# NHLBI/long_context_biomedical_imaging

Hardware: AMD Instinct MI355X
Metric: image-tokens/sec fwd+bwd, ViT patch=2 512^2 (L=65536), 1/2/4/8 MI355X (higher is better)
Workload: dtype bf16; 1 GPU; ViT-small p2 512x512 2-D seg (ViTUNETR head), full attention; global_batch=2, seq_len=65536, parallelism=ddp1, per_gpu_batch=2, optimizer=adam, loss=CrossEntropy, activation_checkpointing=none, hip_graph=False, tuned_gemms=True

## Files before the change

### include/lci.h

```cpp
#ifndef LCI_H_
#define LCI_H_

#ifdef __cplusplus
extern "C" {
#endif

#define LCI_ABI_VERSION 40
const char* lci_last_error(void);
int lci_abi_version(void);
const char* lci_build_hash(void);

int lci_attn_fwd(const void* qkv, void* out, float* lse2, float* knorm_ws, int B, int L, int H, int head_dim,
                 float scale, void* stream);
long long lci_attn_fwd_ws_bytes(int B, int L, int H);
int lci_attn_fwd_variant(int variant, const void* qkv, void* out, float* lse2, float* knorm_ws, int B, int L, int H,
                         int head_dim, float scale, void* stream);
int lci_attn_fwd_pick(int B, int L, int H, int n_cu);
int lci_attn_bwd(const void* qkv, const void* out, const void* dout, const float* lse2, void* dqkv,
                 float* delta_ws, int B, int L, int H, int head_dim, float scale, void* stream);
long long lci_attn_bwd_ws_bytes(int B, int H, int L);
int lci_attn_bwd_stage(int stage, const void* qkv, const void* out, const void* dout, const float* lse2,
                       void* dqkv, float* delta_ws, int B, int L, int H, int head_dim, float scale, void* stream);
int lci_attn_bwd_variant(int dq_variant, int stage, const void* qkv, const void* out, const void* dout,
                         const float* lse2, void* dqkv, float* delta_ws, int B, int L, int H, int head_dim,
                         float scale, void* stream);
int lci_attn_bwd_dq_pick(int B, int L, int H, int n_cu);

int lci_attn_gen_fwd(int dtype, const void* qkv, void* out, float* lse, int B, int L, int H, int head_dim,
                     float scale, void* stream);
int lci_attn_gen_bwd(int dtype, const void* qkv, const void* out, const void* dout, const float* lse, void* dqkv,
                     float* delta_ws, int B, int L, int H, int head_dim, float scale, void* stream);

long long lci_window_bias_elems(const int* geo, int has_mask);
int lci_window_bias(const float* rpb, const float* mask, void* bias, void* biasT, const int* geo, void* stream);
int lci_window_attn_fwd(const void* qkv, const float* qkv_bias, const void* biasT, int has_mask, void* out,
                        float* lse2, const int* geo, float scale, void* stream);
int lci_window_attn_bwd(const void* qkv, const float* qkv_bias, const void* bias, const void* biasT, int has_mask,
                        const void* out, const void* dout, const float* lse2, void* dqkv, float* dbias_pad,
                        float* pad_ws, void* dS, float* drpb, const int* geo, float scale, void* stream);
long long lci_window_dS_elems(const int* geo);
long long lci_window_pad_ws_elems(const int* geo);
int lci_window_bwd_needs_plain(const int* geo);
int lci_window_index_map(const int* geo, int* src_row, int* region, int* rid, int* wtype, void* stream);

int lci_window_gather(const void* src, void* dst, int elem_bytes, const int* geo, int scatter, void* stream);

int lci_conv3_fwd(const void* x, const void* w, void* y, int B, int D, int H, int W, int Cin, int Cout, int KD,
                  void* stream);
int lci_conv3_fwd_splits(long long V, int Cin, int Cout, int KD);
int lci_conv3_pack_weight(const float* w, void* out, int Cout, int Cin, int KD, int mode, int Cin_pad, void* stream);
int lci_convup_interleave(const void* src, void* dst, int B, int D, int H, int W, int kd, int kh, int kw, int C, int ld,
                          int adjoint, void* stream);
int lci_conv3_fwd_split(const void* x, const void* w, void* y, float* part, int nsplit, int B, int D, int H, int W,
                        int Cin, int Cout, int KD, void* stream);
long long lci_conv3_wgrad_splits(long long V, int Cin, int Cout, int KD);
int lci_conv3_wgrad(const void* x, const void* dy, float* part, int B, int D, int H, int W, int Cin, int Cout,
                    int KD, void* stream);

int lci_inorm_chunks(long long V, int B);
int lci_inorm_reduce(const void* x, const void* dz, const float* stats, float* part, long long V, int B, int C,
                     int act, float slope, void* stream);
int lci_inorm_finalize(const float* part, float* out, long long V, int B, int C, int mode, float eps, void* stream);
int lci_bn_relu_fwd(const void* x, const float* stats, const float* w, const float* b, float* y, long long V, int C,
                    void* stream);
int lci_bn_relu_bwd_reduce(const void* x, const void* dy, int dy_f32, const float* stats, const float* w,
                           const float* b, float* part, long long V, int C, void* stream);
int lci_bn_relu_bwd_apply(const void* x, const void* dy, int dy_f32, const float* stats, const float* coef,
                          const float* w, const float* b, void* dx, long long V, int C, void* stream);
int lci_inorm_apply(const void* x, const void* dz, const float* stats, const float* coef, void* out, long long V,
                    int B, int C, int act, float slope, void* stream);
int lci_inorm_apply_res(const void* x, const float* stats, const void* y, const float* stats_y, void* out,
                        long long V, int B, int C, float slope, void* stream);

int lci_selective_scan_fwd(int dtype, const void* u, const void* delta, const float* A, const void* Bm,
                           const void* Cm, const float* D, const float* delta_bias, void* y,
                           const long long* strides, int B, int L, int Dx, int N, int chunk, int delta_softplus,
                           float* xend, float* xinit, float* sdt, void* ckpt, void* stream);
int lci_selective_scan_bwd(int dtype, const void* u, const void* delta, const float* A, const void* Bm,
                           const void* Cm, const float* D, const float* delta_bias, const void* dy, void* du,
// ... 149 lines not shown
```

### long_context_biomedical_imaging_amd/csrc/attention.hip

```cpp
#include "common.hpp"

#include <type_traits>
#include <utility>

namespace lci {

constexpr int DH = 64;
constexpr int KT = 64;
constexpr float NEG_BIG = -1.0e30f;

struct AttnArgs {
  const bf16* q; const bf16* k; const bf16* v;
  const bf16* o; const bf16* dout;
  bf16* out;
  bf16* dk; bf16* dv;
  float* lse2;
  float* delta;
  long long bs_q, bs_k, bs_v, bs_o, bs_do, bs_out, bs_dk, bs_dv;
  int rs_q, rs_k, rs_v, rs_o, rs_do, rs_out, rs_dk, rs_dv;
  int hs;
  int H, L;
  float c;
  float scale;
};

__global__ __launch_bounds__(256) void attn_key_norm_kernel(AttnArgs a, float* knorm, int nkt) {
  const int lane = threadIdx.x & 63, t = blockIdx.x * 4 + (threadIdx.x >> 6);
  const int hh = blockIdx.y, b = blockIdx.z;
  if (t >= nkt) return;
  const int key = t * KT + lane;
  float ss = 0.f;
  if (key < a.L) {
    const bf16* kp = a.k + b * a.bs_k + (long long)key * a.rs_k + hh * a.hs;
#pragma unroll
    for (int c = 0; c < DH / 8; ++c) {
      const bf16x8 v = *(const bf16x8*)(kp + 8 * c);
#pragma unroll
      for (int j = 0; j < 8; ++j) ss += to_f32(v[j]) * to_f32(v[j]);
    }
  }
#pragma unroll
  for (int off = 32; off >= 1; off >>= 1) ss = fmaxf(ss, __shfl_xor(ss, off));
  if (lane == 0) knorm[((long long)b * a.H + hh) * nkt + t] = sqrtf(ss);
}

constexpr float SAFE_EXP2 = 64.f;
__global__ __launch_bounds__(256) void attn_bwd_delta_kernel(AttnArgs a) {
  const int tid = threadIdx.x;
  const int row = blockIdx.x * 32 + (tid >> 3), ch = tid & 7;
  const int hh = blockIdx.y, b = blockIdx.z;
  float acc = 0.f;
  if (row < a.L) {
    const bf16x8 o = *(const bf16x8*)(a.o + b * a.bs_o + (long long)row * a.rs_o + hh * a.hs + ch * 8);
    const bf16x8 d = *(const bf16x8*)(a.dout + b * a.bs_do + (long long)row * a.rs_do + hh * a.hs + ch * 8);
#pragma unroll
    for (int j = 0; j < 8; ++j) acc += to_f32(o[j]) * to_f32(d[j]);
  }
  acc += __shfl_xor(acc, 1);
  acc += __shfl_xor(acc, 2);
  acc += __shfl_xor(acc, 4);
  if (ch == 0 && row < a.L) {
    float* ws = a.delta + ((long long)b * a.H + hh) * 2 * a.L;
    ws[row] = -a.lse2[((long long)b * a.H + hh) * a.L + row];
    ws[a.L + row] = -acc;
  }
}

constexpr int HS_NW = 4;
__device__ __forceinline__ int sw128(int row, int col) {
  const int g = ((row >> 2) & 3) | (((row >> 1) & 1) << 2);
  return row * DH + ((((col >> 3) ^ g) << 3) | (col & 7));
}
__device__ __forceinline__ void hs_dma16(rsrc_t r, int voff, int soff, unsigned lds) {
  unsigned keep;
  asm volatile("s_mov_b32 %0, m0\n\ts_mov_b32 m0, %3\n\ts_nop 0\n\tbuffer_load_dwordx4 %1, %2, %4 offen lds\n\ts_mov_b32 m0, %0"
               : "=&s"(keep) : "v"(voff), "s"(r), "s"(lds), "s"(soff) : "memory");
}
__device__ __forceinline__ void hs_dma4(rsrc_t r, int voff, int soff, unsigned lds) {
  unsigned keep;
  asm volatile("s_mov_b32 %0, m0\n\ts_mov_b32 m0, %3\n\ts_nop 0\n\tbuffer_load_dword %1, %2, %4 offen lds\n\ts_mov_b32 m0, %0"
               : "=&s"(keep) : "v"(voff), "s"(r), "s"(lds), "s"(soff) : "memory");
}
__device__ __forceinline__ u32x4 hs_ld16(rsrc_t r, int voff, int soff) {
  u32x4 v;
  asm volatile("buffer_load_dwordx4 %0, %1, %2, %3 offen" : "=a"(v) : "v"(voff), "s"(r), "s"(soff) : "memory");
  return v;
}
__device__ __forceinline__ uint32_t hs_ld4(rsrc_t r, int voff, int soff) {
  uint32_t v;
  asm volatile("buffer_load_dword %0, %1, %2, %3 offen" : "=a"(v) : "v"(voff), "s"(r), "s"(soff) : "memory");
  return v;
}
template <int N>
__device__ __forceinline__ void hs_vmcnt() {
  __builtin_amdgcn_s_waitcnt((N & 15) | ((N >> 4) << 14) | (7 << 4) | (15 << 8));
}
#define HS_TO_AGPR(x) asm volatile("" : "=a"(x) : "0"(x))
#define HS_OPAQUE(x) asm volatile("" : "+v"(x))
#define HS_KEEP(x) asm volatile("" ::"v"(x))
#define HS_EXP(x) asm volatile("v_exp_f32 %0, %0" : "+v"(x))
#define HS_MUL(p, e) asm volatile("v_mul_f32 %0, %1, %0" : "+v"(p) : "v"(e))
#define HS_CVT(w, x0, x1) asm volatile("v_cvt_pk_bf16_f32 %0, %1, %2" : "=v"(w) : "v"(x0), "v"(x1))
#define HS_MFMA_G(acc, A, B) \
  asm volatile("v_mfma_f32_32x32x16_bf16 %0, %1, %2, %0" : "+a"(acc) : "v"(A), "v"(B))
#define HS_MFMA_C0(d, A, B, C) \
  asm volatile("v_mfma_f32_32x32x16_bf16 %0, %1, %2, %3" : "=&v"(d) : "v"(A), "a"(B), "v"(C))
#define HS_MFMA_C(d, A, B) \
  asm volatile("v_mfma_f32_32x32x16_bf16 %0, %1, %2, %0" : "+v"(d) : "v"(A), "a"(B))

constexpr unsigned LGKM0_WAIT = 0xC07F;
template <int OFF>
__device__ __forceinline__ void hs_st16(unsigned addr, const u32x4& v) {
  asm volatile("ds_write_b128 %0, %1 offset:%2" ::"v"(addr), "a"(v), "i"(OFF) : "memory");
}
template <int OFF>
__device__ __forceinline__ void hs_st4(unsigned addr, uint32_t v) {
  asm volatile("ds_write_b32 %0, %1 offset:%2" ::"v"(addr), "a"(v), "i"(OFF) : "memory");
}
__device__ __forceinline__ u32x4 hs_ld16v(rsrc_t r, int voff, int soff) {
  u32x4 v;
  asm volatile("buffer_load_dwordx4 %0, %1, %2, %3 offen" : "=v"(v) : "v"(voff), "s"(r), "s"(soff) : "memory");
  return v;
}
template <int OFF>
__device__ __forceinline__ void hs_st16v(unsigned addr, const u32x4& v) {
  asm volatile("ds_write_b128 %0, %1 offset:%2" ::"v"(addr), "v"(v), "i"(OFF) : "memory");
}
template <class F, int... G>
__device__ __forceinline__ void hs_for_gaps(F&& f, std::integer_sequence<int, G...>) {
  (f(std::integral_constant<int, G>{}), ...);
}

constexpr int HS_TILE_B = KT * DH * 2;
constexpr int HS_SLOT_B = 2 * HS_TILE_B;
constexpr int HS_NSLOT = 4;
static_assert((HS_NSLOT & (HS_NSLOT - 1)) == 0, "ring slot of tile t is t & (HS_NSLOT - 1)");
static_assert(HS_NSLOT * HS_SLOT_B == 65536, "ring reachable by DS immediates");

struct HsRing {
  rsrc_t rx, ry;
  int x0, x1, y0, y1;
  int rs2x, rs2y;
  unsigned lds0;
  int wave;
  static __device__ __forceinline__ int toff(int t, int rs2) { return (int)((uint32_t)t * KT * (uint32_t)rs2); }
  __device__ __forceinline__ rsrc_t rsrc(int i) const { return i < 2 ? rx : ry; }
  __device__ __forceinline__ int voff(int i) const { return i == 0 ? x0 : i == 1 ? x1 : i == 2 ? y0 : y1; }
  __device__ __forceinline__ int soff(int t, int i) const { return toff(t, i < 2 ? rs2x : rs2y); }
  __device__ __forceinline__ void dma(int t, int i) const {
    const unsigned sb = lds0 + (unsigned)((t & (HS_NSLOT - 1)) * HS_SLOT_B);
    hs_dma16(rsrc(i), voff(i), soff(t, i), sb + (i >> 1) * HS_TILE_B + 2048 * wave + (i & 1) * 1024);
  }
};
__device__ __forceinline__ rsrc_t hs_rows_rsrc(const bf16* p, int rs2, int L) {
  return make_rsrc(p, (uint32_t)(L - 1) * (uint32_t)rs2 + DH * 2);
}
__device__ __forceinline__ HsRing hs_ring(rsrc_t rx, int rs2x, rsrc_t ry, int rs2y, int lane, int wave,
                                          const char* smem) {
  HsRing r;
  r.rx = rx;
  r.ry = ry;
// ... 7 lines not shown
  r.lds0 = (unsigned)(uintptr_t)(LCI_LDS char*)smem;
  r.wave = wave;
  return r;
}

__device__ __forceinline__ void hs_load_b2(bf16x8 (&xf)[4], bf16x8 (&yf)[4], const bf16* xp, int rs_x, const bf16* yp,
                                           int rs_y, int row, int L, int h, float c) {
#pragma unroll
  for (int ks = 0; ks < 4; ++ks) {
    if (row < L) {
      xf[ks] = *(const bf16x8*)(xp + (long long)row * rs_x + 16 * ks + 8 * h);
      yf[ks] = *(const bf16x8*)(yp + (long long)row * rs_y + 16 * ks + 8 * h);
    } else {
      xf[ks] = bf16x8{};
      yf[ks] = bf16x8{};
    }
#pragma unroll
    for (int j = 0; j < 8; ++j) xf[ks][j] = to_bf16(to_f32(xf[ks][j]) * c);
  }
}
#ifndef LCI_DKDV_PROBE
#define LCI_DKDV_PROBE 0
#endif
#ifndef LCI_DKDV_DPPRC
#define LCI_DKDV_DPPRC 0
#endif
template <int I>
__device__ __forceinline__ float hs_bcast(float x) {
  float d;
  asm volatile("v_mov_b32_dpp %0, %1 row_newbcast:%2 row_mask:0xf bank_mask:0xf" : "=v"(d) : "v"(x), "i"(I));
  return d;
}
__device__ __forceinline__ float hs_bcast_i(float x, int i) {
  switch (i & 15) {
    case 0: return hs_bcast<0>(x); case 1: return hs_bcast<1>(x); case 2: return hs_bcast<2>(x);
    case 3: return hs_bcast<3>(x); case 4: return hs_bcast<4>(x); case 5: return hs_bcast<5>(x);
    case 6: return hs_bcast<6>(x); case 7: return hs_bcast<7>(x); case 8: return hs_bcast<8>(x);
    case 9: return hs_bcast<9>(x); case 10: return hs_bcast<10>(x); case 11: return hs_bcast<11>(x);
    case 12: return hs_bcast<12>(x); case 13: return hs_bcast<13>(x); case 14: return hs_bcast<14>(x);
    default: return hs_bcast<15>(x);
  }
}
__global__ __launch_bounds__(HS_NW * 64, 1) void attn_bwd_dkdv_hs_kernel(AttnArgs a) {
  constexpr bool DPPRC = LCI_DKDV_DPPRC != 0;
  constexpr int RC_B = 2 * KT * 4;
  constexpr int NOPS = 5;
  __shared__ __attribute__((aligned(16))) char smem[HS_NSLOT * HS_SLOT_B + HS_NSLOT * RC_B];
  char* const rcs = smem + HS_NSLOT * HS_SLOT_B;
  const int tid = threadIdx.x, lane = tid & 63;
  const int wave = __builtin_amdgcn_readfirstlane(tid >> 6);
  const int hh = blockIdx.y, b = blockIdx.z;
  const int L = a.L;
  const int h = lane >> 5, r32 = lane & 31;
  const int kw0 = blockIdx.x * (HS_NW * 64) + wave * 64;
  const int nqt = (L + KT - 1) / KT;

  bf16x8 kf[2][4], vf[2][4];
  {
    const bf16* kp = a.k + b * a.bs_k + hh * a.hs;
    const bf16* vp = a.v + b * a.bs_v + hh * a.hs;
#pragma unroll
    for (int kb = 0; kb < 2; ++kb) {
      hs_load_b2(kf[kb], vf[kb], kp, a.rs_k, vp, a.rs_v, kw0 + 32 * kb + r32, L, h, a.c);
    }
  }
  hs_vmcnt<0>();
#pragma unroll
  for (int i = 0; i < 2; ++i)
#pragma unroll
    for (int j = 0; j < 4; ++j)
      { HS_TO_AGPR(kf[i][j]); HS_TO_AGPR(vf[i][j]); }

  const int rs2q = a.rs_q * 2, rs2d = a.rs_do * 2;
  const rsrc_t rq = hs_rows_rsrc(a.q + b * a.bs_q + hh * a.hs, rs2q, L);
  const rsrc_t rd = hs_rows_rsrc(a.dout + b * a.bs_do + hh * a.hs, rs2d, L);
  const rsrc_t rr = make_rsrc(a.delta + ((long long)b * a.H + hh) * 2 * L + (wave & 1) * L, (uint32_t)L * 4);
  const HsRing ring = hs_ring(rq, rs2q, rd, rs2d, lane, wave, smem);
  const unsigned lds0 = ring.lds0;
  auto dma_op = [&](int t, int i) __attribute__((always_inline)) {
    if (i < 4) ring.dma(t, i);
    if (i == 4) hs_dma4(rr, lane * 4, t * KT * 4,
                        lds0 + (unsigned)(HS_NSLOT * HS_SLOT_B + (t & (HS_NSLOT - 1)) * RC_B + (wave & 1) * KT * 4));
  };
  auto dma_tile = [&](int t) __attribute__((always_inline)) {
#pragma unroll
    for (int i = 0; i < NOPS; ++i) dma_op(t, i);
  };
  unsigned q_off[4], t_off[2][2], rc_off;
#pragma unroll
  for (int ks = 0; ks < 4; ++ks) {
    q_off[ks] = 2 * sw128(r32, 16 * ks + 8 * h);
    HS_OPAQUE(q_off[ks]);
  }
#pragma unroll
  for (int db = 0; db < 2; ++db)
#pragma unroll
    for (int part = 0; part < 2; ++part) {
      t_off[db][part] = 2 * sw128(4 * h + ((lane & 15) >> 2) + 8 * part, 32 * db + 16 * ((lane >> 4) & 1) + 4 * (lane & 3));
      HS_OPAQUE(t_off[db][part]);
    }
  rc_off = HS_NSLOT * HS_SLOT_B + 16 * h;
  HS_OPAQUE(rc_off);
  unsigned rcx_off = HS_NSLOT * HS_SLOT_B + 4 * ((lane & 3) + 8 * ((lane >> 2) & 3) + 4 * h);
  HS_OPAQUE(rcx_off);
  auto qrow = [&](int soff, int r0, int ks) __attribute__((always_inline)) {
    return *(const bf16x8*)(smem + q_off[ks] + (soff + 2 * DH * r0));
  };
// ... 188 lines not shown
        }
      }
      if (seg == LS) {
        ld_piece(t + 2, g >> 1);
        if (g == 7) ld_piece(t + 2, 4);
      }
    };
    auto none = []() __attribute__((always_inline)) {};
    auto nogap = [](int, int) __attribute__((always_inline)) {};
    half(std::integral_constant<int, 0>{}, slot, 0, slot, rc, 32, none, rstg0);
    half(std::integral_constant<int, 1>{}, slot, 32, nslot, nrc, 0, stage, nogap);
  };
  int t = 0;
  for (; t + 4 <= nqt; t += 4) {
    tile(std::integral_constant<int, 0>{}, t);
    tile(std::integral_constant<int, 1>{}, t + 1);
    tile(std::integral_constant<int, 2>{}, t + 2);
    tile(std::integral_constant<int, 3>{}, t + 3);
  }
  for (; t < nqt; ++t) tile(std::integral_constant<int, -1>{}, t);
  hs_vmcnt<0>();
#pragma unroll
  for (int g = 0; g < 8; ++g) valu_gap(g, 1, 1, 1, 0);
  HS_MUL(P[1][14], S[1][14]);
  HS_MUL(P[1][15], S[1][15]);
  asm volatile("s_nop 0" ::: "memory");
  HS_CVT(pk[1][1][3], S[1][14], S[1][15]);
  HS_CVT(dd[1][1][2], P[1][12], P[1][13]);
  HS_CVT(dd[1][1][3], P[1][14], P[1][15]);
  asm volatile("s_nop 1" ::: "memory");
#pragma unroll
  for (int g = 0; g < 8; ++g) grad_gap(g, 1, 1);
  asm volatile("s_nop 15\n\ts_nop 15\n\ts_nop 15\n\ts_nop 15" ::: "memory");

  const float sc = a.scale;
#pragma unroll
  for (int kb = 0; kb < 2; ++kb) {
    const int key = kw0 + 32 * kb + r32;
    if (key < L) {
      bf16* dkp = a.dk + b * a.bs_dk + (long long)key * a.rs_dk + hh * a.hs;
      bf16* dvp = a.dv + b * a.bs_dv + (long long)key * a.rs_dv + hh * a.hs;
#pragma unroll
      for (int db = 0; db < 2; ++db)
#pragma unroll
        for (int g = 0; g < 4; ++g) {
          bf16x4 k4, v4;
#pragma unroll
          for (int j = 0; j < 4; ++j) {
            k4[j] = to_bf16(dk[db][kb][4 * g + j] * sc);
            v4[j] = to_bf16(dv[db][kb][4 * g + j]);
          }
          *(bf16x4*)(dkp + 32 * db + 8 * g + 4 * h) = k4;
          *(bf16x4*)(dvp + 32 * db + 8 * g + 4 * h) = v4;
        }
    }
  }
}

constexpr unsigned char DQ_SCHED[24][4] = {
    {0x28, 0x29, 0xff, 0xff},
    {0x68, 0x69, 0x2a, 0xa4},
    {0x6a, 0x2b, 0x2c, 0xff},
    {0x6b, 0x6c, 0xa5, 0x2d},
    {0x2e, 0x6d, 0x2f, 0xa6},
    {0x6e, 0x6f, 0x00, 0xa7},
    {0x01, 0x02, 0xff, 0xff},
    {0x03, 0x04, 0xff, 0xff},
    {0x05, 0x06, 0xff, 0xff},
    {0x40, 0x41, 0x42, 0x43},
    {0x80, 0x81, 0x44, 0x45},
    {0x46, 0x82, 0x07, 0x08},
    {0x47, 0x48, 0x83, 0x09},
    {0x0a, 0x49, 0x0b, 0x84},
    {0x4a, 0x4b, 0x0c, 0x85},
    {0x4c, 0x0d, 0x0e, 0xff},
    {0x4d, 0x4e, 0x86, 0x0f},
    {0x20, 0x4f, 0x21, 0x87},
    {0x22, 0x23, 0xff, 0xff},
    {0x24, 0x25, 0xff, 0xff},
    {0x26, 0x27, 0xff, 0xff},
    {0x60, 0x61, 0x62, 0x63},
    {0xa0, 0xa1, 0x64, 0x65},
    {0x66, 0x67, 0xa2, 0xa3}};


#ifndef LCI_DQ_EARLY
#define LCI_DQ_EARLY 1
#endif
constexpr bool DQ_EARLY = LCI_DQ_EARLY != 0;
__device__ __forceinline__ void attn_bwd_dq_hs_body(const AttnArgs& a) {
  __shared__ __attribute__((aligned(16))) char smem[HS_NSLOT * HS_SLOT_B];
  const int tid = threadIdx.x, lane = tid & 63;
  const int wave = __builtin_amdgcn_readfirstlane(tid >> 6);
  const int hh = blockIdx.y, b = blockIdx.z;
  const int L = a.L;
  const int h = lane >> 5, r32 = lane & 31;
  const int qw0 = blockIdx.x * (HS_NW * 64) + wave * 64;
  const int nkt = (L + KT - 1) / KT;
  const int nkt4 = (nkt + 3) & ~3;

  bf16x8 qf[2][4], df[2][4];
  f32x16 NL[2], ND[2];
  {
    const bf16* qp = a.q + b * a.bs_q + hh * a.hs;
    const bf16* dop = a.dout + b * a.bs_do + hh * a.hs;
    const float* ws = a.delta + ((long long)b * a.H + hh) * 2 * L;
// ... 1441 lines not shown
  if (B <= 0 || L <= 0 || H <= 0 || n_cu <= 0) return 0;
  const long long W = (long long)B * H * ((L + qwg - 1) / qwg);
  if (W < n_cu) return 0;
  const long long rounds = (W + n_cu - 1) / n_cu;
  return 10 * W >= 9 * rounds * n_cu ? 1 : 0;
}
extern "C" int lci_attn_fwd_pick(int B, int L, int H, int n_cu) { return attn_wide_pick(B, L, H, n_cu, FW4_QWG); }
extern "C" int lci_attn_bwd_dq_pick(int B, int L, int H, int n_cu) { return attn_wide_pick(B, L, H, n_cu, DQ4_QWG); }

static int attn_n_cu() {
  static const int n = [] {
    int dev = 0, cu = 0;
    if (hipGetDevice(&dev) != hipSuccess ||
        hipDeviceGetAttribute(&cu, hipDeviceAttributeMultiprocessorCount, dev) != hipSuccess)
      return 0;
    return cu;
  }();
  return n;
}

extern "C" int lci_attn_fwd_variant(int variant, const void* qkv, void* out, float* lse2, float* knorm_ws, int B,
                                    int L, int H, int head_dim, float scale, void* stream) {
  LCI_CHECK(variant >= -1 && variant <= 1, "lci_attn_fwd_variant: variant %d (want -1, 0 or 1)", variant);
  if (attn_check("lci_attn_fwd", qkv, nullptr, out, nullptr, B, L, H, head_dim)) return 1;
  LCI_CHECK(knorm_ws != nullptr, "lci_attn_fwd: knorm_ws (lci_attn_fwd_ws_bytes) is required");
  AttnArgs a = attn_args(qkv, L, H, scale);
  a.out = (bf16*)out; a.lse2 = lse2;
  a.bs_out = (long long)L * H * DH; a.rs_out = H * DH;
  hipStream_t s = (hipStream_t)stream;
  const int nkt = (L + KT - 1) / KT;
  hipLaunchKernelGGL(attn_key_norm_kernel, dim3((nkt + 3) / 4, H, B), dim3(256), 0, s, a, knorm_ws, nkt);
  LCI_LAUNCH_CHECK();
  if (variant < 0) variant = lci_attn_fwd_pick(B, L, H, attn_n_cu());
  if (variant == 1)
    hipLaunchKernelGGL(attn_fwd_hs4_kernel, dim3((L + FW4_QWG - 1) / FW4_QWG, H, B), dim3(HS_NW * 64), 0, s, a,
                       (const float*)knorm_ws);
  else
    hipLaunchKernelGGL(attn_fwd_hs_kernel, dim3((L + HS_NW * 64 - 1) / (HS_NW * 64), H, B), dim3(HS_NW * 64), 0, s, a,
                       (const float*)knorm_ws);
  LCI_LAUNCH_CHECK();
  return 0;
}

extern "C" int lci_attn_fwd(const void* qkv, void* out, float* lse2, float* knorm_ws, int B, int L, int H,
                            int head_dim, float scale, void* stream) {
  return lci_attn_fwd_variant(-1, qkv, out, lse2, knorm_ws, B, L, H, head_dim, scale, stream);
}

extern "C" long long lci_attn_bwd_ws_bytes(int B, int H, int L) {
  const long long flags = (long long)B * H * ((L + DQ4_QWG - 1) / DQ4_QWG);
  return ((dq4_flag_offset(B, H, L) + flags) * 4 + 255) / 256 * 256;
}

extern "C" int lci_attn_bwd_variant(int dq_variant, int stage, const void* qkv, const void* out, const void* dout,
                                    const float* lse2, void* dqkv, float* delta_ws, int B, int L, int H, int head_dim,
                                    float scale, void* stream) {
  LCI_CHECK(dq_variant >= -1 && dq_variant <= 1, "lci_attn_bwd_variant: dq_variant %d (want -1, 0 or 1)", dq_variant);
  if (attn_check("lci_attn_bwd", qkv, dqkv, out, dout, B, L, H, head_dim)) return 1;
  LCI_CHECK(delta_ws != nullptr, "lci_attn_bwd: delta_ws (lci_attn_bwd_ws_bytes) is required");
  AttnArgs a = attn_args(qkv, L, H, scale);
  bf16* dbase = (bf16*)dqkv;
  a.o = (const bf16*)out; a.dout = (const bf16*)dout;
  a.lse2 = (float*)lse2; a.delta = delta_ws;
  a.bs_o = a.bs_do = (long long)L * H * DH;
  a.rs_o = a.rs_do = H * DH;
  a.out = dbase; a.dk = dbase + H * DH; a.dv = dbase + 2 * H * DH;
  a.bs_out = a.bs_dk = a.bs_dv = a.bs_q;
  a.rs_out = a.rs_dk = a.rs_dv = a.rs_q;
  hipStream_t s = (hipStream_t)stream;
  const dim3 grid((L + HS_NW * 64 - 1) / (HS_NW * 64), H, B);
  if (stage < 0 || stage == 0) {
    hipLaunchKernelGGL(attn_bwd_delta_kernel, dim3((L + 31) / 32, H, B), dim3(256), 0, s, a);
    LCI_LAUNCH_CHECK();
  }
  if (stage < 0 || stage == 1) {
    hipLaunchKernelGGL(attn_bwd_dkdv_hs_kernel, grid, dim3(HS_NW * 64), 0, s, a);
    LCI_LAUNCH_CHECK();
  }
  if (stage < 0 || stage == 2) {
    if (dq_variant < 0) dq_variant = lci_attn_bwd_dq_pick(B, L, H, attn_n_cu());
    if (dq_variant == 1) {
      hipLaunchKernelGGL(attn_bwd_dq_hs4_kernel, dim3((L + DQ4_QWG - 1) / DQ4_QWG, H, B), dim3(HS_NW * 64), 0, s, a);
      LCI_LAUNCH_CHECK();
      hipLaunchKernelGGL(attn_bwd_dq_hsfb_kernel, grid, dim3(HS_NW * 64), 0, s, a);
    } else {
      hipLaunchKernelGGL(attn_bwd_dq_hs_kernel, grid, dim3(HS_NW * 64), 0, s, a);
    }
    LCI_LAUNCH_CHECK();
  }
  return 0;
}

extern "C" int lci_attn_bwd_stage(int stage, const void* qkv, const void* out, const void* dout, const float* lse2,
                                  void* dqkv, float* delta_ws, int B, int L, int H, int head_dim, float scale,
                                  void* stream) {
  return lci_attn_bwd_variant(-1, stage, qkv, out, dout, lse2, dqkv, delta_ws, B, L, H, head_dim, scale, stream);
}

extern "C" int lci_attn_bwd(const void* qkv, const void* out, const void* dout, const float* lse2, void* dqkv,
                            float* delta_ws, int B, int L, int H, int head_dim, float scale, void* stream) {
  return lci_attn_bwd_stage(-1, qkv, out, dout, lse2, dqkv, delta_ws, B, L, H, head_dim, scale, stream);
}
```

### long_context_biomedical_imaging_amd/kernels.py

```python
from __future__ import annotations

import ctypes
import os

import torch

from . import _lib


class KernelTimer:
    enabled = False
    only = None
    records: list = []

    @classmethod
    def run(cls, name, work, t, fn):
        if not cls.enabled or (cls.only is not None and name not in cls.only):
            fn()
            return
        st = torch.cuda.current_stream(t.device)
        e0, e1 = torch.cuda.Event(enable_timing=True), torch.cuda.Event(enable_timing=True)
        e0.record(st)
        fn()
        e1.record(st)
# ... 27 lines not shown
    out = torch.empty(B, L, num_heads * dh, device=qkv.device, dtype=torch.bfloat16)
    lse2 = torch.empty(B, num_heads, L, device=qkv.device, dtype=torch.float32)
    ws = torch.empty(_lib.load().lci_attn_fwd_ws_bytes(B, L, num_heads) // 4, device=qkv.device, dtype=torch.float32)
    return B, L, dh, out, lse2, ws


def attn_fwd(qkv: torch.Tensor, num_heads: int, scale: float):
    B, L, dh, out, lse2, ws = _attn_fwd_setup(qkv, num_heads, "attn_fwd")
    KernelTimer.run("attn_fwd", 4.0 * B * num_heads * L * L * dh, qkv, lambda: _lib.call(
        "lci_attn_fwd", qkv.data_ptr(), out.data_ptr(), lse2.data_ptr(), ws.data_ptr(), B, L, num_heads, dh,
        float(scale), _lib.stream_of(qkv)))
    return out, lse2


def attn_fwd_variant(qkv: torch.Tensor, num_heads: int, scale: float, variant: int):
    B, L, dh, out, lse2, ws = _attn_fwd_setup(qkv, num_heads, "attn_fwd_variant")
    _lib.call("lci_attn_fwd_variant", int(variant), qkv.data_ptr(), out.data_ptr(), lse2.data_ptr(), ws.data_ptr(), B,
              L, num_heads, dh, float(scale), _lib.stream_of(qkv))
    return out, lse2


def _attn_bwd_setup(qkv, out, dout, lse2, num_heads: int, scale: float, dqkv=None, ws=None):
    _lib.require_gpu(qkv, out, dout, lse2)
    B, L, C = qkv.shape
    dh = C // (3 * num_heads)
    if dqkv is None:
        dqkv = torch.empty_like(qkv)
    if ws is None:
        ws = torch.empty(int(_lib.load().lci_attn_bwd_ws_bytes(B, num_heads, L)) // 4, device=qkv.device,
                         dtype=torch.int32)
    args = (qkv.data_ptr(), out.data_ptr(), dout.data_ptr(), lse2.data_ptr(), dqkv.data_ptr(), ws.data_ptr(),
            B, L, num_heads, dh, float(scale), _lib.stream_of(qkv))
    return B, L, dh, dqkv, ws, args


def attn_bwd(qkv, out, dout, lse2, num_heads: int, scale: float):
    B, L, dh, dqkv, _, args = _attn_bwd_setup(qkv, out, dout, lse2, num_heads, scale)
    if not KernelTimer.enabled:
        _lib.call("lci_attn_bwd", *args)
        return dqkv
    f = float(B) * num_heads * L * L * dh
    KernelTimer.run("attn_bwd_delta", 0.0, qkv, lambda: _lib.call("lci_attn_bwd_stage", 0, *args))
    KernelTimer.run("attn_bwd_dkdv", 6.0 * f, qkv, lambda: _lib.call("lci_attn_bwd_stage", 1, *args))
    KernelTimer.run("attn_bwd_dq", 2.0 * f, qkv, lambda: _lib.call("lci_attn_bwd_stage", 2, *args))
    return dqkv


def attn_bwd_variant(qkv, out, dout, lse2, num_heads: int, scale: float, dq_variant: int, stage: int = -1, ws=None,
                     dqkv=None):
    B, L, _, dqkv, ws, args = _attn_bwd_setup(qkv, out, dout, lse2, num_heads, scale, dqkv, ws)
    _lib.call("lci_attn_bwd_variant", int(dq_variant), int(stage), *args)
    n0, nwg = B * num_heads * 2 * L, (L + 511) // 512
    return dqkv, ws[n0:n0 + B * num_heads * nwg].view(B, num_heads, nwg)


class _FlashAttention(torch.autograd.Function):
    @staticmethod
    def forward(ctx, qkv, num_heads, scale):
        out, lse2 = attn_fwd(qkv, num_heads, scale)
        ctx.save_for_backward(qkv, out, lse2)
        ctx.num_heads, ctx.scale = num_heads, scale
        return out

    @staticmethod
    def backward(ctx, dout):
        qkv, out, lse2 = ctx.saved_tensors
        dout = dout.to(torch.bfloat16).contiguous()
        return attn_bwd(qkv, out, dout, lse2, ctx.num_heads, ctx.scale), None, None


ATTN_HEAD_DIM = 64
ATTN_GEN_MAX_HEAD_DIM = 256
WIN_HEAD_DIM = 32


def attn_gen_fwd(qkv: torch.Tensor, num_heads: int, scale: float):
    _lib.require_gpu(qkv)
    B, L, C = qkv.shape
    dh = C // (3 * num_heads)
    out = torch.empty(B, L, num_heads * dh, device=qkv.device, dtype=qkv.dtype)
    lse = torch.empty(B, num_heads, L, device=qkv.device, dtype=torch.float32)
    KernelTimer.run("attn_gen_fwd", 4.0 * B * num_heads * L * L * dh, qkv, lambda: _lib.call(
        "lci_attn_gen_fwd", _lib.DTYPE[qkv.dtype], qkv.data_ptr(), out.data_ptr(), lse.data_ptr(), B, L, num_heads, dh,
        float(scale), _lib.stream_of(qkv)))
    return out, lse


def attn_gen_bwd(qkv, out, dout, lse, num_heads: int, scale: float):
    _lib.require_gpu(qkv, out, dout, lse)
    B, L, C = qkv.shape
    dh = C // (3 * num_heads)
    dqkv = torch.empty_like(qkv)
    delta = torch.empty(B, num_heads, L, device=qkv.device, dtype=torch.float32)
    KernelTimer.run("attn_gen_bwd", 8.0 * B * num_heads * L * L * dh, qkv, lambda: _lib.call(
        "lci_attn_gen_bwd", _lib.DTYPE[qkv.dtype], qkv.data_ptr(), out.data_ptr(), dout.data_ptr(), lse.data_ptr(),
        dqkv.data_ptr(), delta.data_ptr(), B, L, num_heads, dh, float(scale), _lib.stream_of(qkv)))
    return dqkv


class _GenAttention(torch.autograd.Function):
    @staticmethod
    def forward(ctx, qkv, num_heads, scale):
        out, lse = attn_gen_fwd(qkv, num_heads, scale)
        ctx.save_for_backward(qkv, out, lse)
        ctx.num_heads, ctx.scale = num_heads, scale
        return out
# ... 2170 lines not shown
```

Baseline: 227,700 image-tokens/s.

## Add 96-key-per-wave dK/dV backward kernel with wide/narrow grid split

Adds a dK/dV backward kernel in which each wave holds 96 keys instead of 64. The third key block lives in VGPRs, because AGPRs are already taken by the first two blocks. Each streamed Q/dO tile is therefore reused across more keys, which cuts LDS/DMA traffic and loop overhead per key. A cost model picks how many wide workgroups to launch, and the original kernel covers the remaining keys from a new k0 offset. The cost is higher register pressure and two launches, and the heuristic may pick zero wide workgroups for some shapes.

```diff
diff --git a/include/lci.h b/include/lci.h
--- a/include/lci.h
+++ b/include/lci.h
@@ -5,7 +5,7 @@
 extern "C" {
 #endif
 
-#define LCI_ABI_VERSION 40
+#define LCI_ABI_VERSION 41
 const char* lci_last_error(void);
 int lci_abi_version(void);
 const char* lci_build_hash(void);
@@ -25,6 +25,10 @@
                          const float* lse2, void* dqkv, float* delta_ws, int B, int L, int H, int head_dim,
                          float scale, void* stream);
 int lci_attn_bwd_dq_pick(int B, int L, int H, int n_cu);
+int lci_attn_bwd_variant2(int dq_variant, int dkdv_wide_wgs, int stage, const void* qkv, const void* out,
+                          const void* dout, const float* lse2, void* dqkv, float* delta_ws, int B, int L, int H,
+                          int head_dim, float scale, void* stream);
+int lci_attn_bwd_dkdv_pick(int B, int L, int H, int n_cu);
 
 int lci_attn_gen_fwd(int dtype, const void* qkv, void* out, float* lse, int B, int L, int H, int head_dim,
                      float scale, void* stream);
diff --git a/long_context_biomedical_imaging_amd/csrc/attention.hip b/long_context_biomedical_imaging_amd/csrc/attention.hip
--- a/long_context_biomedical_imaging_amd/csrc/attention.hip
+++ b/long_context_biomedical_imaging_amd/csrc/attention.hip
@@ -22,6 +22,7 @@
   int H, L;
   float c;
   float scale;
+  int k0;
 };
 
 __global__ __launch_bounds__(256) void attn_key_norm_kernel(AttnArgs a, float* knorm, int nkt) {
@@ -107,6 +108,10 @@
   asm volatile("v_mfma_f32_32x32x16_bf16 %0, %1, %2, %3" : "=&v"(d) : "v"(A), "a"(B), "v"(C))
 #define HS_MFMA_C(d, A, B) \
   asm volatile("v_mfma_f32_32x32x16_bf16 %0, %1, %2, %0" : "+v"(d) : "v"(A), "a"(B))
+#define HS_MFMA_C0V(d, A, B, C) \
+  asm volatile("v_mfma_f32_32x32x16_bf16 %0, %1, %2, %3" : "=&v"(d) : "v"(A), "v"(B), "v"(C))
+#define HS_MFMA_CV(d, A, B) \
+  asm volatile("v_mfma_f32_32x32x16_bf16 %0, %1, %2, %0" : "+v"(d) : "v"(A), "v"(B))
 
 constexpr unsigned LGKM0_WAIT = 0xC07F;
 template <int OFF>
@@ -220,7 +225,7 @@
   const int hh = blockIdx.y, b = blockIdx.z;
   const int L = a.L;
   const int h = lane >> 5, r32 = lane & 31;
-  const int kw0 = blockIdx.x * (HS_NW * 64) + wave * 64;
+  const int kw0 = a.k0 + blockIdx.x * (HS_NW * 64) + wave * 64;
   const int nqt = (L + KT - 1) / KT;
 
   bf16x8 kf[2][4], vf[2][4];
@@ -515,6 +520,298 @@
           }
           *(bf16x4*)(dkp + 32 * db + 8 * g + 4 * h) = k4;
           *(bf16x4*)(dvp + 32 * db + 8 * g + 4 * h) = v4;
+        }
+    }
+  }
+}
+
+constexpr int DKV3_KWG = HS_NW * 96;
+__global__ __launch_bounds__(HS_NW * 64, 1) void attn_bwd_dkdv_hs3_kernel(AttnArgs a) {
+  constexpr int RC_B = 2 * KT * 4;
+  constexpr int NOPS = 5;
+  __shared__ __attribute__((aligned(16))) char smem[HS_NSLOT * HS_SLOT_B + HS_NSLOT * RC_B];
+  char* const rcs = smem + HS_NSLOT * HS_SLOT_B;
+  const int tid = threadIdx.x, lane = tid & 63;
+  const int wave = __builtin_amdgcn_readfirstlane(tid >> 6);
+  const int hh = blockIdx.y, b = blockIdx.z;
+  const int L = a.L;
+  const int h = lane >> 5, r32 = lane & 31;
+  const int kw0 = blockIdx.x * DKV3_KWG + wave * 96;
+  const int nqt = (L + KT - 1) / KT;
+
+  bf16x8 kf[3][4], vf[3][4];
+  {
+    const bf16* kp = a.k + b * a.bs_k + hh * a.hs;
+    const bf16* vp = a.v + b * a.bs_v + hh * a.hs;
+#pragma unroll
+    for (int kb = 0; kb < 3; ++kb) {
+      hs_load_b2(kf[kb], vf[kb], kp, a.rs_k, vp, a.rs_v, kw0 + 32 * kb + r32, L, h, a.c);
+    }
+  }
+  hs_vmcnt<0>();
+#pragma unroll
+  for (int j = 0; j < 4; ++j) {
+    HS_TO_AGPR(kf[0][j]); HS_TO_AGPR(vf[0][j]);
+    HS_TO_AGPR(kf[1][j]); HS_TO_AGPR(vf[1][j]);
+    HS_OPAQUE(kf[2][j]); HS_OPAQUE(vf[2][j]);
+  }
+
+  const int rs2q = a.rs_q * 2, rs2d = a.rs_do * 2;
+  const rsrc_t rq = hs_rows_rsrc(a.q + b * a.bs_q + hh * a.hs, rs2q, L);
+  const rsrc_t rd = hs_rows_rsrc(a.dout + b * a.bs_do + hh * a.hs, rs2d, L);
+  const rsrc_t rr = make_rsrc(a.delta + ((long long)b * a.H + hh) * 2 * L + (wave & 1) * L, (uint32_t)L * 4);
+  const HsRing ring = hs_ring(rq, rs2q, rd, rs2d, lane, wave, smem);
+  const unsigned lds0 = ring.lds0;
+  auto dma_op = [&](int t, int i) __attribute__((always_inline)) {
+    if (i < 4) ring.dma(t, i);
+    if (i == 4) hs_dma4(rr, lane * 4, t * KT * 4,
+                        lds0 + (unsigned)(HS_NSLOT * HS_SLOT_B + (t & (HS_NSLOT - 1)) * RC_B + (wave & 1) * KT * 4));
+  };
+  unsigned q_off[4], t_off[2][2], rc_off;
+#pragma unroll
+  for (int ks = 0; ks < 4; ++ks) {
+    q_off[ks] = 2 * sw128(r32, 16 * ks + 8 * h);
+    HS_OPAQUE(q_off[ks]);
+  }
+#pragma unroll
+  for (int db = 0; db < 2; ++db)
+#pragma unroll
+    for (int part = 0; part < 2; ++part) {
+      t_off[db][part] = 2 * sw128(4 * h + ((lane & 15) >> 2) + 8 * part, 32 * db + 16 * ((lane >> 4) & 1) + 4 * (lane & 3));
+      HS_OPAQUE(t_off[db][part]);
+    }
+  rc_off = HS_NSLOT * HS_SLOT_B + 16 * h;
+  HS_OPAQUE(rc_off);
+  auto qrow = [&](int soff, int r0, int ks) __attribute__((always_inline)) {
+    return *(const bf16x8*)(smem + q_off[ks] + (soff + 2 * DH * r0));
+  };
+  auto trf = [&](int soff, int r0, int S, int db) __attribute__((always_inline)) {
+    const int imm = soff + 2 * DH * (r0 + 16 * S);
+    return cat44(lds_tr4((const bf16*)(smem + t_off[db][0] + imm)), lds_tr4((const bf16*)(smem + t_off[db][1] + imm)));
+  };
+  auto rcblk = [&](const char* rcslot, int which, int r0) __attribute__((always_inline)) {
+    const float* rc = (const float*)(rcslot + which * KT * 4) + r0 + 4 * h;
+    f32x16 r;
+#pragma unroll
+    for (int g = 0; g < 4; ++g) {
+      const f32x4 v = *(const f32x4*)(rc + 8 * g);
+      r[4 * g] = v[0]; r[4 * g + 1] = v[1]; r[4 * g + 2] = v[2]; r[4 * g + 3] = v[3];
+    }
+    return r;
+  };
+
+  f32x16 dv[2][3], dk[2][3];
+  f32x16 S[2], P[2];
+  f32x16 NLs, NDs;
+#pragma unroll
+  for (int i = 0; i < 2; ++i) {
+    S[i] = P[i] = f32x16{};
+#pragma unroll
+    for (int j = 0; j < 3; ++j) dv[i][j] = dk[i][j] = f32x16{};
+  }
+  u32x4 pk[2][2] = {}, dd[2][2] = {};
+  bf16x8 tdo[2][2] = {}, tq[2][2] = {};
+#pragma unroll
+  for (int i = 0; i < 2; ++i) {
+    HS_OPAQUE(S[i]);
+    HS_OPAQUE(P[i]);
+#pragma unroll
+    for (int j = 0; j < 3; ++j) {
+      HS_TO_AGPR(dv[i][j]);
+      HS_TO_AGPR(dk[i][j]);
+    }
+#pragma unroll
+    for (int j = 0; j < 2; ++j) {
+      HS_OPAQUE(pk[i][j]);
+      HS_OPAQUE(dd[i][j]);
+      HS_OPAQUE(tdo[i][j]);
+      HS_OPAQUE(tq[i][j]);
+    }
+  }
+  bf16x8 qa[4], da[4];
+
+  auto valu_gap = [&](int g, int st, int e, int pst, int pe) __attribute__((always_inline)) {
+    f32x16& s = S[st];
+    f32x16& p = P[st];
+    const int o = 8 * e, po = 8 * pe;
+    HS_EXP(s[o + g]);
+    if (g >= 2) HS_MUL(p[o + g - 2], s[o + g - 2]);
+    if (g == 0) HS_MUL(P[pst][po + 6], S[pst][po + 6]);
+    if (g == 1) HS_MUL(P[pst][po + 7], S[pst][po + 7]);
+    switch (g) {
+      case 0: HS_CVT(pk[pst][pe][3], S[pst][po + 6], S[pst][po + 7]); break;
+      case 1: HS_CVT(dd[pst][pe][2], P[pst][po + 4], P[pst][po + 5]); break;
+      case 2: HS_CVT(dd[pst][pe][3], P[pst][po + 6], P[pst][po + 7]); break;
+      case 3: HS_CVT(pk[st][e][0], s[o], s[o + 1]); break;
+      case 4: HS_CVT(pk[st][e][1], s[o + 2], s[o + 3]); break;
+      case 5: HS_CVT(dd[st][e][0], p[o], p[o + 1]); break;
+      case 6: HS_CVT(pk[st][e][2], s[o + 4], s[o + 5]); break;
+      default: HS_CVT(dd[st][e][1], p[o + 2], p[o + 3]); break;
+    }
+  };
+  auto chain_gap = [&](int g, int kb, int st) __attribute__((always_inline)) {
+    if (kb < 2) {
+      if (g == 0) HS_MFMA_C0(S[st], qa[0], kf[kb][0], NLs);
+      else if (g < 4) HS_MFMA_C(S[st], qa[g], kf[kb][g]);
+      else if (g == 4) HS_MFMA_C0(P[st], da[0], vf[kb][0], NDs);
+      else HS_MFMA_C(P[st], da[g - 4], vf[kb][g - 4]);
+    } else {
+      if (g == 0) HS_MFMA_C0V(S[st], qa[0], kf[2][0], NLs);
+      else if (g < 4) HS_MFMA_CV(S[st], qa[g], kf[2][g]);
+      else if (g == 4) HS_MFMA_C0V(P[st], da[0], vf[2][0], NDs);
+      else HS_MFMA_CV(P[st], da[g - 4], vf[2][g - 4]);
+    }
+  };
+  auto grad_gap = [&](int g, int kb, int st) __attribute__((always_inline)) {
+    const int s2 = g >> 2, db = (g >> 1) & 1;
+    const bf16x8 pb = __builtin_bit_cast(bf16x8, pk[st][s2]);
+    const bf16x8 db8 = __builtin_bit_cast(bf16x8, dd[st][s2]);
+    if (g & 1) HS_MFMA_G(dk[db][kb], tq[db][s2], db8);
+    else HS_MFMA_G(dv[db][kb], tdo[db][s2], pb);
+  };
+  auto tr_load = [&](int f, int soff, int r0) __attribute__((always_inline)) {
+    const int s2 = f >> 2, db = (f >> 1) & 1;
+    if (f & 1) tq[db][s2] = trf(soff, r0, s2, db);
+    else tdo[db][s2] = trf(soff + HS_TILE_B, r0, s2, db);
+  };
+  auto rc_load = [&](f32x16& r, int rcoff, int which, int r0, int g) __attribute__((always_inline)) {
+    const f32x4 v = *(const f32x4*)(smem + rc_off + (rcoff + which * KT * 4 + 4 * (r0 + 8 * g)));
+    r[4 * g] = v[0]; r[4 * g + 1] = v[1]; r[4 * g + 2] = v[2]; r[4 * g + 3] = v[3];
+  };
+
+  auto half = [&](auto CUR, int slot, int r0, int nslot, int nrc, int nr0, auto mid, auto sgap)
+      __attribute__((always_inline)) {
+    constexpr int X = decltype(CUR)::value, Y = X ^ 1;
+#pragma unroll
+    for (int g = 0; g < 8; ++g) {
+      chain_gap(g, 0, X);
+      valu_gap(g, Y, 1, Y, 0);
+      sgap(0, g);
+    }
+    mid();
+#pragma unroll
+    for (int g = 0; g < 8; ++g) {
+      grad_gap(g, 2, Y);
+      valu_gap(g, X, 0, Y, 1);
+      if (g >= 2) tr_load(g - 2, slot, r0);
+      sgap(1, g);
+    }
+#pragma unroll
+    for (int g = 0; g < 8; ++g) {
+      chain_gap(g, 1, Y);
+      valu_gap(g, X, 1, X, 0);
+      if (g < 2) tr_load(6 + g, slot, r0);
+      sgap(2, g);
+    }
+#pragma unroll
+    for (int g = 0; g < 8; ++g) {
+      grad_gap(g, 0, X);
+      valu_gap(g, Y, 0, X, 1);
+      sgap(3, g);
+    }
+#pragma unroll
+    for (int g = 0; g < 8; ++g) {
+      chain_gap(g, 2, X);
+      valu_gap(g, Y, 1, Y, 0);
+      if (g == 2) HS_KEEP(NLs);
+      if (g == 6) HS_KEEP(NDs);
+      if (g >= 2 && g < 6) qa[g - 2] = qrow(nslot, nr0, g - 2);
+      if (g >= 6) {
+        rc_load(NLs, nrc, 0, nr0, g - 6);
+        da[g - 6] = qrow(nslot + HS_TILE_B, nr0, g - 6);
+      }
+      sgap(4, g);
+    }
+#pragma unroll
+    for (int g = 0; g < 8; ++g) {
+      grad_gap(g, 1, Y);
+      valu_gap(g, X, 0, Y, 1);
+      if (g < 2) rc_load(NLs, nrc, 0, nr0, g + 2);
+      else if (g < 6) rc_load(NDs, nrc, 1, nr0, g - 2);
+      else da[g - 4] = qrow(nslot + HS_TILE_B, nr0, g - 4);
+      sgap(5, g);
+    }
+  };
+
+#pragma unroll
+  for (int i = 0; i < NOPS; ++i) dma_op(0, i);
+#pragma unroll
+  for (int i = 0; i < NOPS; ++i) dma_op(1, i);
+  hs_vmcnt<0>();
+  __syncthreads();
+  NLs = rcblk(rcs, 0, 0);
+  NDs = rcblk(rcs, 1, 0);
+#pragma unroll
+  for (int ks = 0; ks < 4; ++ks) {
+    qa[ks] = qrow(0, 0, ks);
+    da[ks] = qrow(HS_TILE_B, 0, ks);
+  }
+  __builtin_amdgcn_s_waitcnt(LGKM0_WAIT);
+  auto tile = [&](auto SL, int t) __attribute__((always_inline)) {
+    constexpr int SLC = decltype(SL)::value;
+    const int sl = SLC >= 0 ? SLC : t & (HS_NSLOT - 1);
+    const int nsl = SLC >= 0 ? (SLC + 1) & (HS_NSLOT - 1) : (t + 1) & (HS_NSLOT - 1);
+    const int slot = sl * HS_SLOT_B, nslot = nsl * HS_SLOT_B, nrc = nsl * RC_B;
+    auto stage = [&]() __attribute__((always_inline)) {
+      if (t + 1 < nqt) {
+        hs_vmcnt<NOPS>();
+        __builtin_amdgcn_s_barrier();
+      }
+    };
+    auto rstg0 = [&](int seg, int g) __attribute__((always_inline)) {
+      if (seg != 2 || !(g & 1)) return;
+      dma_op(t + 2, g >> 1);
+      if (g == 7) dma_op(t + 2, 4);
+    };
+    auto none = []() __attribute__((always_inline)) {};
+    auto nogap = [](int, int) __attribute__((always_inline)) {};
+    half(std::integral_constant<int, 0>{}, slot, 0, slot, sl * RC_B, 32, none, rstg0);
+    half(std::integral_constant<int, 1>{}, slot, 32, nslot, nrc, 0, stage, nogap);
+  };
+  int t = 0;
+  for (; t + 4 <= nqt; t += 4) {
+    tile(std::integral_constant<int, 0>{}, t);
+    tile(std::integral_constant<int, 1>{}, t + 1);
+    tile(std::integral_constant<int, 2>{}, t + 2);
+    tile(std::integral_constant<int, 3>{}, t + 3);
+  }
+  for (; t < nqt; ++t) tile(std::integral_constant<int, -1>{}, t);
+  hs_vmcnt<0>();
+#pragma unroll
+  for (int g = 0; g < 8; ++g) valu_gap(g, 1, 1, 1, 0);
+  HS_MUL(P[1][14], S[1][14]);
+  HS_MUL(P[1][15], S[1][15]);
+  asm volatile("s_nop 0" ::: "memory");
+  HS_CVT(pk[1][1][3], S[1][14], S[1][15]);
+  HS_CVT(dd[1][1][2], P[1][12], P[1][13]);
+  HS_CVT(dd[1][1][3], P[1][14], P[1][15]);
+  asm volatile("s_nop 1" ::: "memory");
+#pragma unroll
+  for (int g = 0; g < 8; ++g) grad_gap(g, 2, 1);
+  asm volatile("s_nop 15\n\ts_nop 15\n\ts_nop 15\n\ts_nop 15" ::: "memory");
+
+  int etid = tid;
+  HS_OPAQUE(etid);
+  const int eh = (etid >> 5) & 1, er32 = etid & 31;
+  const float sc = a.scale;
+#pragma unroll
+  for (int kb = 0; kb < 3; ++kb) {
+    const int key = kw0 + 32 * kb + er32;
+    if (key < L) {
+      bf16* dkp = a.dk + b * a.bs_dk + (long long)key * a.rs_dk + hh * a.hs;
+      bf16* dvp = a.dv + b * a.bs_dv + (long long)key * a.rs_dv + hh * a.hs;
+#pragma unroll
+      for (int db = 0; db < 2; ++db)
+#pragma unroll
+        for (int g = 0; g < 4; ++g) {
+          bf16x4 k4, v4;
+#pragma unroll
+          for (int j = 0; j < 4; ++j) {
+            k4[j] = to_bf16(dk[db][kb][4 * g + j] * sc);
+            v4[j] = to_bf16(dv[db][kb][4 * g + j]);
+          }
+          *(bf16x4*)(dkp + 32 * db + 8 * g + 4 * eh) = k4;
+          *(bf16x4*)(dvp + 32 * db + 8 * g + 4 * eh) = v4;
         }
     }
   }
@@ -2062,11 +2359,32 @@
   return ((dq4_flag_offset(B, H, L) + flags) * 4 + 255) / 256 * 256;
 }
 
-extern "C" int lci_attn_bwd_variant(int dq_variant, int stage, const void* qkv, const void* out, const void* dout,
-                                    const float* lse2, void* dqkv, float* delta_ws, int B, int L, int H, int head_dim,
-                                    float scale, void* stream) {
+static bool attn_grid_fills(long long wgs, int n_cu) {
+  return wgs >= n_cu && 10 * wgs >= 9 * ((wgs + n_cu - 1) / n_cu) * n_cu;
+}
+extern "C" int lci_attn_bwd_dkdv_pick(int B, int L, int H, int n_cu) {
+  if (B <= 0 || L <= 0 || H <= 0 || n_cu <= 0) return 0;
+  const long long bh = (long long)B * H;
+  const int nkw = HS_NW * 64;
+  long long best_cost = 2 * ((bh * ((L + nkw - 1) / nkw) + n_cu - 1) / n_cu);
+  int best = 0;
+  for (int W = 1; W <= L / DKV3_KWG; ++W) {
+    const long long wide = bh * W, rest = bh * ((L - DKV3_KWG * W + nkw - 1) / nkw);
+    if (!attn_grid_fills(wide, n_cu) || (rest && !attn_grid_fills(rest, n_cu))) continue;
+    const long long cost = 3 * ((wide + n_cu - 1) / n_cu) + 2 * ((rest + n_cu - 1) / n_cu);
+    if (cost <= best_cost) best_cost = cost, best = W;
+  }
+  return best;
+}
+
+extern "C" int lci_attn_bwd_variant2(int dq_variant, int dkdv_wide_wgs, int stage, const void* qkv, const void* out,
+                                     const void* dout, const float* lse2, void* dqkv, float* delta_ws, int B, int L,
+                                     int H, int head_dim, float scale, void* stream) {
   LCI_CHECK(dq_variant >= -1 && dq_variant <= 1, "lci_attn_bwd_variant: dq_variant %d (want -1, 0 or 1)", dq_variant);
   if (attn_check("lci_attn_bwd", qkv, dqkv, out, dout, B, L, H, head_dim)) return 1;
+  LCI_CHECK(dkdv_wide_wgs >= -1 && (dkdv_wide_wgs <= 0 || (long long)DKV3_KWG * (dkdv_wide_wgs - 1) < L),
+            "lci_attn_bwd_variant2: dkdv_wide_wgs %d (want -1, 0 or at most ceil(L / 384) = %d)", dkdv_wide_wgs,
+            (L + DKV3_KWG - 1) / DKV3_KWG);
   LCI_CHECK(delta_ws != nullptr, "lci_attn_bwd: delta_ws (lci_attn_bwd_ws_bytes) is required");
   AttnArgs a = attn_args(qkv, L, H, scale);
   bf16* dbase = (bf16*)dqkv;
@@ -2084,8 +2402,17 @@
     LCI_LAUNCH_CHECK();
   }
   if (stage < 0 || stage == 1) {
-    hipLaunchKernelGGL(attn_bwd_dkdv_hs_kernel, grid, dim3(HS_NW * 64), 0, s, a);
-    LCI_LAUNCH_CHECK();
+    const int W = dkdv_wide_wgs < 0 ? lci_attn_bwd_dkdv_pick(B, L, H, attn_n_cu()) : dkdv_wide_wgs;
+    if (W > 0) {
+      hipLaunchKernelGGL(attn_bwd_dkdv_hs3_kernel, dim3(W, H, B), dim3(HS_NW * 64), 0, s, a);
+      LCI_LAUNCH_CHECK();
+    }
+    a.k0 = W * DKV3_KWG;
+    if (a.k0 < L) {
+      hipLaunchKernelGGL(attn_bwd_dkdv_hs_kernel, dim3((L - a.k0 + HS_NW * 64 - 1) / (HS_NW * 64), H, B),
+                         dim3(HS_NW * 64), 0, s, a);
+      LCI_LAUNCH_CHECK();
+    }
   }
   if (stage < 0 || stage == 2) {
     if (dq_variant < 0) dq_variant = lci_attn_bwd_dq_pick(B, L, H, attn_n_cu());
@@ -2101,6 +2428,13 @@
   return 0;
 }
 
+extern "C" int lci_attn_bwd_variant(int dq_variant, int stage, const void* qkv, const void* out, const void* dout,
+                                    const float* lse2, void* dqkv, float* delta_ws, int B, int L, int H, int head_dim,
+                                    float scale, void* stream) {
+  return lci_attn_bwd_variant2(dq_variant, -1, stage, qkv, out, dout, lse2, dqkv, delta_ws, B, L, H, head_dim, scale,
+                               stream);
+}
+
 extern "C" int lci_attn_bwd_stage(int stage, const void* qkv, const void* out, const void* dout, const float* lse2,
                                   void* dqkv, float* delta_ws, int B, int L, int H, int head_dim, float scale,
                                   void* stream) {
diff --git a/long_context_biomedical_imaging_amd/kernels.py b/long_context_biomedical_imaging_amd/kernels.py
--- a/long_context_biomedical_imaging_amd/kernels.py
+++ b/long_context_biomedical_imaging_amd/kernels.py
@@ -103,6 +103,13 @@
     _lib.call("lci_attn_bwd_variant", int(dq_variant), int(stage), *args)
     n0, nwg = B * num_heads * 2 * L, (L + 511) // 512
     return dqkv, ws[n0:n0 + B * num_heads * nwg].view(B, num_heads, nwg)
+
+
+def attn_bwd_variant2(qkv, out, dout, lse2, num_heads: int, scale: float, dq_variant: int, dkdv_wide_wgs: int,
+                      stage: int = -1, ws=None, dqkv=None):
+    _, _, _, dqkv, _, args = _attn_bwd_setup(qkv, out, dout, lse2, num_heads, scale, dqkv, ws)
+    _lib.call("lci_attn_bwd_variant2", int(dq_variant), int(dkdv_wide_wgs), int(stage), *args)
+    return dqkv
 
 
 class _FlashAttention(torch.autograd.Function):
```

Result: faster. 232,500 image-tokens/s, median of 6 (+2.1%).
